# AHupuJR/REFID

Hardware: AMD Instinct MI355X
Metric: interpolated frames/sec (train step) GoPro 256x256 11+1 (higher is better)
Workload: dtype f32

## Files before the change

### refid_amd/csrc/conv_wino6.hip

```cpp
#include "common.h"
#include "conv_args.h"
#include <algorithm>
#include <cstdlib>

#ifndef REFID_WINO6_ABLATE
#define REFID_WINO6_ABLATE 0
#endif

namespace {

constexpr int TW = 32;
constexpr int KC = 16;
constexpr int HWD = TW + 2;
constexpr int TH = 4;
constexpr int ROWP = 40;
constexpr int PLANE = 6 * ROWP + 5;
constexpr int R_F4 = 4 * PLANE;
constexpr int HP = (TH + 2) * HWD;
constexpr int R_ITEMS = (4 * HP + 255) / 256;
constexpr int lds_bytes(int nt) { return nt == 2 ? 64 * 66 * 16 : (32 * 66 * 16 > 2 * R_F4 * 16 ? 32 * 66 * 16 : 2 * R_F4 * 16); }
constexpr int OOB = -1;
typedef __bf16 bf16x8 __attribute__((ext_vector_type(8)));
typedef _Float16 f16x8 __attribute__((ext_vector_type(8)));
typedef _Float16 f16x2 __attribute__((ext_vector_type(2)));
typedef float f32x2 __attribute__((ext_vector_type(2)));
constexpr int W3H_HEADER = 64;
constexpr int F16_TGT = 7;
constexpr int F16_SLACK = 6;
constexpr int F16_E0 = F16_TGT + 1;

__device__ __forceinline__ void split8(const f32x4& v0, const f32x4& v1, f32x4 (&pl)[3]) {
    bf16x8 p0, p1, p2;
#pragma unroll
    for (int k = 0; k < 8; ++k) {
        const float v = k < 4 ? v0[k] : v1[k - 4];
        const __bf16 h = (__bf16)v;
        p0[k] = h;
        const float r = v - (float)h;
        const __bf16 m = (__bf16)r;
        p1[k] = m;
        p2[k] = (__bf16)(r - (float)m);
    }
    pl[0] = __builtin_bit_cast(f32x4, p0);
    pl[1] = __builtin_bit_cast(f32x4, p1);
    pl[2] = __builtin_bit_cast(f32x4, p2);
}

__device__ __forceinline__ void split8h(const f32x4& v0, const f32x4& v1, f32x4 (&pl)[3]) {
    f16x8 h, l;
#pragma unroll
    for (int k = 0; k < 8; k += 2) {
        const f32x2 ab = {k < 4 ? v0[k] : v1[k - 4], k < 4 ? v0[k + 1] : v1[k - 3]};
        const f16x2 hh = __builtin_convertvector(ab, f16x2);
        const f32x2 r = ab - __builtin_convertvector(hh, f32x2);
        const f16x2 ll = __builtin_convertvector(r, f16x2);
        h[k] = hh[0]; h[k + 1] = hh[1];
        l[k] = ll[0]; l[k + 1] = ll[1];
    }
    pl[0] = __builtin_bit_cast(f32x4, h);
    pl[1] = __builtin_bit_cast(f32x4, l);
}

template <int NT, bool F16>
__global__ __launch_bounds__(256, NT == 2 ? 2 : 3) void conv_wino6_kernel(const ConvKArgs a) {
    constexpr int BN = 32 * NT;
    constexpr int NPL = F16 ? 2 : 3;
    constexpr int NPR = (REFID_WINO6_ABLATE == 14 || REFID_WINO6_ABLATE == 15) ? 3 : (F16 ? 3 : 6);
    extern __shared__ __attribute__((aligned(16))) char smem[];
    f32x4* sR = reinterpret_cast<f32x4*>(smem);

    const int tid = threadIdx.x;
    const int lane = tid & 63, wave = tid >> 6;
    const int li = lane & 31, kh = lane >> 5;
    const int ti = wave;
    if (REFID_WINO6_ABLATE == 20 && a.N > 0) return;
    if (REFID_WINO6_ABLATE == 21 && a.N > 0) { __syncthreads(); if (tid == 12345) a.out[0] = 1.f; return; }

#if defined(REFID_WINO6_ABLATE) && (REFID_WINO6_ABLATE == 9 || REFID_WINO6_ABLATE == 11)
    {
        unsigned hw;
        asm volatile("s_getreg_b32 %0, hwreg(HW_REG_HW_ID)" : "=s"(hw));
        if ((hw & 1) && blockIdx.x < 512 * 2) {
            const unsigned long long t0 = wall_clock64();
            while (wall_clock64() - t0 < (REFID_WINO6_ABLATE == 9 ? 400 : 800)) __builtin_amdgcn_s_sleep(8);
        }
    }
#endif
    const int xcd = blockIdx.x & 7, slot = blockIdx.x >> 3;
    int bt = (slot / a.ncot) * 8 + xcd;
    if (bt >= a.tilesX * a.tilesY * a.N) return;
    const int n0 = (slot % a.ncot) * BN;
    const int tx = bt % a.tilesX; bt /= a.tilesX;
    const int ty = bt % a.tilesY;
    const int n = bt / a.tilesY;
    const int oy0 = ty * TH, ox0 = tx * TW;

    const int limA = (int)min((long long)a.N * a.H * a.W * a.ldA * 4, 0x7fffffffLL);
    const int limB = a.inB ? (int)min((long long)a.N * a.H * a.W * a.ldB * 4, 0x7fffffffLL) : 0;
    const int uPlane = a.CoutPad * KC * 2;
    const int uXi = NPL * uPlane;
    const int uChunk = 16 * uXi;
    const __amdgpu_buffer_rsrc_t rsW = __builtin_amdgcn_make_buffer_rsrc(
        const_cast<float*>(a.w) + (F16 ? W3H_HEADER / 4 : 0), 0, (int)min((long long)a.nchunks * uChunk, 0x7fffffffLL), 0x00020000);
    const int eU = F16 ? *reinterpret_cast<const int*>(a.w) : 0;
    int eRef = F16_E0;
    const int q = tid & 3;
    int pixo[R_ITEMS], sdst[R_ITEMS];
#pragma unroll
    for (int it = 0; it < R_ITEMS; ++it) {
        const int hp = (tid >> 2) + it * 64;
        const int row = hp / HWD, col = hp % HWD;
        const int iy = oy0 - a.pad + row, ix = ox0 - a.pad + col;
        const bool ok = hp < HP && iy >= 0 && iy < a.H && ix >= 0 && ix < a.W;
        pixo[it] = ok ? (n * a.H + iy) * a.W + ix : OOB;
        sdst[it] = hp < HP ? q * PLANE + row * ROWP + (col >> 1) + (col & 1) * 20 : q * PLANE + 6 * ROWP + (tid & 3);
    }
    int voU[NT];
#pragma unroll
    for (int nt = 0; nt < NT; ++nt) {
        const int urow = a.coBase + n0 + nt * 32 + li;
        voU[nt] = (urow < a.CoutPad) ? (urow * KC + kh * 8) * 2 + ti * 4 * uXi : OOB;
        if (REFID_WINO6_ABLATE == 12) voU[nt] = ti * 4 * uXi;
    }
    const int kper = (a.nchunks + a.ksplit - 1) / a.ksplit;
    const int kc0 = blockIdx.y * kper, kc1 = min(a.nchunks, kc0 + kper);

    f32x4 rr[R_ITEMS];
    auto load_raw = [&](int ch, f32x4 (&dst)[R_ITEMS]) {
        const int c0 = (REFID_WINO6_ABLATE == 5 ? 0 : ch) * KC;
        const bool fromA = c0 < a.Ca;
        const int soff = (fromA ? c0 : c0 - a.Ca) * 4;
        const int qmask = (ch < kc1 && c0 + q * 4 < a.Ctot) ? 0 : OOB;
        const int ld4 = (fromA ? a.ldA : a.ldB) * 4;
        const __amdgpu_buffer_rsrc_t rs = __builtin_amdgcn_make_buffer_rsrc(
            const_cast<float*>(fromA ? a.inA : a.inB), 0, fromA ? limA : limB, 0x00020000);
#pragma unroll
        for (int it = 0; it < R_ITEMS; ++it) {
            const int vo = (pixo[it] * ld4 + q * 16) | qmask;
            dst[it] = __builtin_bit_cast(f32x4, __builtin_amdgcn_raw_buffer_load_b128(rs, vo, soff, 0));
        }
    };
    auto store_raw = [&](int buf, const f32x4 (&src)[R_ITEMS]) {
#pragma unroll
        for (int it = 0; it < R_ITEMS; ++it) sR[buf * R_F4 + sdst[it]] = src[it];
    };
    auto load_u = [&](int ch, int j, f32x4 (&dst)[NPL][NT]) {
        const bool in = ch < kc1;
        const int so = (REFID_WINO6_ABLATE == 1 ? 0 : ch) * uChunk + j * uXi;
#pragma unroll
        for (int p = 0; p < ((REFID_WINO6_ABLATE == 14 || REFID_WINO6_ABLATE == 15) ? 2 : NPL); ++p)
#pragma unroll
            for (int nt = 0; nt < NT; ++nt) {
                if (REFID_WINO6_ABLATE == 13 && nt == 1) { dst[p][nt] = dst[p][0]; continue; }
                dst[p][nt] = __builtin_bit_cast(
                    f32x4, __builtin_amdgcn_raw_buffer_load_b128(rsW, in ? voU[nt] : OOB, in ? so + p * uPlane : 0, 0));
            }
    };

    f32x16 acc[4][NT];
#pragma unroll
    for (int j = 0; j < 4; ++j)
#pragma unroll
        for (int t = 0; t < NT; ++t)
#pragma unroll
            for (int r = 0; r < 16; ++r) acc[j][t][r] = 0.f;

    const int rowP = (ti == 0) ? 0 : ((ti == 2) ? 2 : 1);
    const int rowM = (ti == 0) ? 2 : ((ti == 1) ? 2 : ((ti == 2) ? 1 : 3));
    const float sgn = (ti == 1) ? 1.f : -1.f;
    const int tbase = 2 * kh * PLANE + (2 * (li >> 4)) * ROWP + (li & 15);
    const int offP = tbase + rowP * ROWP, offM = tbase + rowM * ROWP;
    constexpr int BOFF[4] = {0, 20, 1, 21};

    constexpr int TA[6] = {0, 0, 1, 0, 2, 1};
    constexpr int TB[6] = {0, 1, 0, 2, 0, 1};

    f32x4 uA[NPL][NT], uB[NPL][NT];
    auto phase = [&](int ch) {
        const int lc = ch - kc0;
        if (REFID_WINO6_ABLATE != 7 && REFID_WINO6_ABLATE != 8) {
            store_raw((lc + 1) & 1, rr);
            load_raw(ch + 2, rr);
#ifdef REFID_WINO6_PIN
            __builtin_amdgcn_sched_barrier(0x38F);
#endif
        }
        const f32x4* r = sR + (lc & 1) * R_F4;
        f32x4 t[2][4];
#pragma unroll
        for (int qq = 0; qq < 2; ++qq)
#pragma unroll
            for (int b = 0; b < 4; ++b) t[qq][b] = r[qq * PLANE + offP + BOFF[b]] + r[qq * PLANE + offM + BOFF[b]] * sgn;
        if constexpr (F16 && REFID_WINO6_ABLATE != 16) {
            float m = 0.f;
#pragma unroll
            for (int qq = 0; qq < 2; ++qq)
#pragma unroll
                for (int b = 0; b < 4; ++b)
                    m = fmaxf(fmaxf(m, fmaxf(fabsf(t[qq][b][0]), fabsf(t[qq][b][1]))), fmaxf(fabsf(t[qq][b][2]), fabsf(t[qq][b][3])));
            if (REFID_WINO6_ABLATE == 17) m = fabsf(t[0][0][0]);
            const unsigned mb = __float_as_uint(m);
            const auto sw = __builtin_amdgcn_permlane32_swap(mb, mb, false, false);
            const int eb = (int)(max(sw[0], sw[1]) >> 23);
            const bool grow = eb > eRef + F16_SLACK;
            if (__builtin_amdgcn_ballot_w64(grow) != 0) {
                const int en = grow ? eb : eRef;
                const int fe = 127 + eRef - en;
                const float f = fe >= 1 ? __uint_as_float((unsigned)fe << 23) : 0.f;
#pragma unroll
                for (int j = 0; j < 4; ++j)
#pragma unroll
                    for (int nt = 0; nt < NT; ++nt)
#pragma unroll
                        for (int rr2 = 0; rr2 < 16; ++rr2) acc[j][nt][rr2] *= f;
                eRef = en;
            }
            const float sc = __uint_as_float((unsigned)(F16_TGT + 254 - eRef) << 23);
#pragma unroll
            for (int qq = 0; qq < 2; ++qq)
#pragma unroll
                for (int b = 0; b < 4; ++b) t[qq][b] *= sc;
        }
#pragma unroll
        for (int j = 0; j < 4; ++j) {
            f32x4 (&cur)[NPL][NT] = (j & 1) ? uB : uA;
            f32x4 (&nxt)[NPL][NT] = (j & 1) ? uA : uB;
            if (REFID_WINO6_ABLATE != 6 && REFID_WINO6_ABLATE != 8) load_u(j == 3 ? ch + 1 : ch, (j + 1) & 3, nxt);
#ifdef REFID_WINO6_PIN
            __builtin_amdgcn_sched_barrier(0x38F);
#endif
            f32x4 v[2], pl[3];
#pragma unroll
            for (int qq = 0; qq < 2; ++qq)
                v[qq] = (j == 0) ? t[qq][0] - t[qq][2] : (j == 1) ? t[qq][1] + t[qq][2]
                      : (j == 2) ? t[qq][2] - t[qq][1] : t[qq][1] - t[qq][3];
            if (REFID_WINO6_ABLATE == 2 || REFID_WINO6_ABLATE == 15) { pl[0] = v[0]; pl[1] = v[1]; pl[2] = t[0][j]; }
            else if (F16 && REFID_WINO6_ABLATE == 18) { pl[0] = v[0]; pl[1] = v[1]; }
            else if constexpr (F16) split8h(v[0], v[1], pl);
            else split8(v[0], v[1], pl);
#pragma unroll
            for (int e = 0; e < NPR; ++e)
#pragma unroll
                for (int nt = 0; nt < NT; ++nt) {
                    if constexpr (F16)
                        acc[j][nt] = __builtin_amdgcn_mfma_f32_32x32x16_f16(
                            __builtin_bit_cast(f16x8, cur[TB[e]][nt]), __builtin_bit_cast(f16x8, pl[TA[e]]), acc[j][nt], 0, 0, 0);
                    else
                        acc[j][nt] = __builtin_amdgcn_mfma_f32_32x32x16_bf16(
                            __builtin_bit_cast(bf16x8, cur[TB[e]][nt]), __builtin_bit_cast(bf16x8, pl[TA[e]]), acc[j][nt], 0, 0, 0);
                }
        }
        __syncthreads();
    };

    {
        f32x4 rr0[R_ITEMS];
#if REFID_WINO6_ABLATE == 19
        int keep[R_ITEMS];
#pragma unroll
        for (int it = 0; it < R_ITEMS; ++it) {
            keep[it] = pixo[it];
            const int hp = (tid >> 2) + it * 64;
            const int row = hp / HWD, col = hp % HWD;
            pixo[it] = (hp < HP && row >= a.pad && col >= a.pad) ? (row - a.pad) * a.W + (col - a.pad) : OOB;
        }
#endif
        load_raw(kc0, rr0);
        load_raw(kc0 + 1, rr);
#if REFID_WINO6_ABLATE == 19
#pragma unroll
        for (int it = 0; it < R_ITEMS; ++it) pixo[it] = keep[it];
#endif
        load_u(kc0, 0, uA);
        if (REFID_WINO6_ABLATE == 6 || REFID_WINO6_ABLATE == 8) load_u(kc0, 1, uB);
        store_raw(0, rr0);
    }
    __syncthreads();

    if (REFID_WINO6_ABLATE != 3 && REFID_WINO6_ABLATE != 10)
        for (int ch = kc0; ch < kc1; ++ch) phase(ch);

    constexpr int XL = 66;
    f32x4* xch = reinterpret_cast<f32x4*>(smem);
#pragma unroll
    for (int t = 0; t < NT; ++t)
#pragma unroll
        for (int rq = 0; rq < 4; ++rq) {
            f32x4 r0, r1;
#pragma unroll
            for (int k = 0; k < 4; ++k) {
                const int r = 4 * rq + k;
                r0[k] = acc[0][t][r] + acc[1][t][r] + acc[2][t][r];
                r1[k] = acc[1][t][r] - acc[2][t][r] - acc[3][t][r];
                if constexpr (F16) {
                    r0[k] = ldexpf(r0[k], eRef - 127 - F16_TGT - eU);
                    r1[k] = ldexpf(r1[k], eRef - 127 - F16_TGT - eU);
                }
            }
            xch[(((ti * 2 + 0) * NT + t) * 4 + rq) * XL + kh * 33 + li] = r0;
            xch[(((ti * 2 + 1) * NT + t) * 4 + rq) * XL + kh * 33 + li] = r1;
        }
    constexpr int QUADS = BN / 4, PPT = 256 / QUADS, CPR = TW / PPT;
    constexpr int NIT = TH * CPR;
    static_assert(TW == 32 && (NT == 1 || NT == 2) && PPT * CPR == TW, "epilogue item mapping");
    constexpr int TI_STRIDE = 2 * NT * 4 * XL;
    const int p0 = tid / QUADS, c = (tid % QUADS) * 4;
    const int j0 = n0 + c;
    const int nt = c >> 5, rq = (c & 31) >> 3, ckh = (c & 7) >> 2;
    const long long opb = (long long)(n * a.Ho + oy0) * a.Wo + ox0 + p0;
    const bool jok = j0 < a.Cout;
    const bool vec = a.vecOK && (j0 + 3 < a.Cout);
    bool cok[CPR];
#pragma unroll
    for (int q2 = 0; q2 < CPR; ++q2) cok[q2] = ox0 + q2 * PPT + p0 < a.Wo;
    float* const outB = a.out + (a.ksplit > 1 ? blockIdx.y * a.wsStride : 0) + opb * a.ldO + j0;
    const float* const resB = a.res ? a.res + opb * a.ldR + j0 : nullptr;
    const float* const mskB = a.mask ? a.mask + opb * a.ldM + j0 : nullptr;
    const int stepO[2] = {a.Wo * a.ldO, PPT * a.ldO}, stepR[2] = {a.Wo * a.ldR, PPT * a.ldR}, stepM[2] = {a.Wo * a.ldM, PPT * a.ldM};
    const bool two = a.out2 != nullptr && a.ksplit == 1;
    float* const out2B = two ? a.out2 + opb * a.ldO2 + j0 : nullptr;
    const float* const add2B = two ? a.add2 + opb * a.ldA2 + j0 : nullptr;
    const int stepO2[2] = {a.Wo * a.ldO2, PPT * a.ldO2}, stepA2[2] = {a.Wo * a.ldA2, PPT * a.ldA2};
    const bool pre = REFID_WINO6_ABLATE != 4 && REFID_WINO6_ABLATE != 10 && vec && a.ksplit == 1 && (a.res != nullptr || a.mask != nullptr);
    f32x4 pres[NIT], pmask[NIT];
    if (pre) {
#pragma unroll
        for (int it = 0; it < NIT; ++it) {
            const bool ok = (oy0 + it / CPR < a.Ho) && cok[it % CPR];
            pres[it] = f32x4{0.f, 0.f, 0.f, 0.f};
            pmask[it] = f32x4{1.f, 1.f, 1.f, 1.f};
            if (ok && a.res) pres[it] = *reinterpret_cast<const f32x4*>(resB + (it / CPR) * stepR[0] + (it % CPR) * stepR[1]);
            if (ok && a.mask) pmask[it] = *reinterpret_cast<const f32x4*>(mskB + (it / CPR) * stepM[0] + (it % CPR) * stepM[1]);
        }
    }
    f32x4 bv = {0.f, 0.f, 0.f, 0.f};
    if (a.bias && a.ksplit == 1 && jok) {
        const float* bp = a.bias + a.coBase + j0;
        if (vec) bv = *reinterpret_cast<const f32x4*>(bp);
        else
#pragma unroll
            for (int k = 0; k < 4; ++k) if (j0 + k < a.Cout) bv[k] = bp[k];
    }
    __syncthreads();

#pragma unroll
    for (int it = 0; it < NIT; ++it) {
        const int row = it / CPR, colb = it % CPR;
        const int col = colb * PPT + p0;
        const int oa = row & 1, tile = ((row & 3) >> 1) * 16 + (col >> 1), ob = col & 1;
        if (oy0 + row >= a.Ho || !cok[colb] || !jok) continue;
        const f32x4* xp = xch + (((oa * 2 + ob) * NT + nt) * 4 + rq) * XL + ckh * 33 + tile;
        const float sg = oa ? -1.f : 1.f;
        f32x4 v = xp[0] + (xp[TI_STRIDE] + xp[2 * TI_STRIDE]) * sg;
        float* const outp = outB + row * stepO[0] + colb * stepO[1];
        if (a.ksplit > 1) {
            *reinterpret_cast<f32x4*>(outp) = v;
            continue;
        }
        v += bv;
        lrelu4(v, a.slopePre, a.slopePre != 1.f);
        if (REFID_WINO6_ABLATE == 4 || REFID_WINO6_ABLATE == 10) {
            if (v[0] == 12345.678f) outp[0] = v[1];
            continue;
        }
        if (vec) {
            if (a.res) v += pre ? pres[it] : *reinterpret_cast<const f32x4*>(resB + row * stepR[0] + colb * stepR[1]);
            lrelu4(v, a.slopePost, a.slopePost != 1.f);
            if (a.mask) {
                const f32x4 mv = pre ? pmask[it] : *reinterpret_cast<const f32x4*>(mskB + row * stepM[0] + colb * stepM[1]);
#pragma unroll
                for (int k = 0; k < 4; ++k) v[k] *= (mv[k] > 0.f) ? 1.f : a.slopeMask;
            }
            *reinterpret_cast<f32x4*>(outp) = v;
            if (two)
                *reinterpret_cast<f32x4*>(out2B + row * stepO2[0] + colb * stepO2[1]) =
                    v + *reinterpret_cast<const f32x4*>(add2B + row * stepA2[0] + colb * stepA2[1]);
        } else {
#pragma unroll
            for (int k = 0; k < 4; ++k) {
                if (j0 + k >= a.Cout) break;
                float tv = v[k];
                if (a.res) tv += resB[row * stepR[0] + colb * stepR[1] + k];
                tv = lrelu(tv, a.slopePost);
                if (a.mask) tv *= (mskB[row * stepM[0] + colb * stepM[1] + k] > 0.f) ? 1.f : a.slopeMask;
                outp[k] = tv;
                if (two) out2B[row * stepO2[0] + colb * stepO2[1] + k] = tv + add2B[row * stepA2[0] + colb * stepA2[1] + k];
            }
        }
    }
}

struct Wino6Plan { int ks; int nt; dim3 grid; };

Wino6Plan wino6_plan(ConvKArgs& a, int split_mode, int tile_hint = 0) {
    Wino6Plan p;
    p.nt = (a.Cout > 32 && tile_hint != 4) ? 2 : 1;
    a.tilesX = cdiv(a.Wo, TW);
    a.tilesY = cdiv(a.Ho, TH);
    if (p.nt == 2 && tile_hint == 0 && split_mode) {
        const int ncot2 = cdiv(a.Cout, 64);
        const int nwg2 = (split_mode == 2) ? round_up(a.tilesX * a.tilesY * a.N, 8) * ncot2 : a.tilesX * a.tilesY * ncot2 * 8;
        static const int small_wg = []() { const char* e = getenv("REFID_WINO6_SMALL"); return e ? atoi(e) : 512; }();
        static const int small_k = []() { const char* e = getenv("REFID_WINO6_SMALL_K"); return e ? atoi(e) : 9; }();
        if (nwg2 <= small_wg && cdiv(a.Ctot, KC) < small_k) p.nt = 1;
    }
    const int bn = 32 * p.nt;
    a.nchunks = cdiv(a.Ctot, KC);
    a.ncot = cdiv(a.Cout, bn);
    p.grid = dim3(round_up(a.tilesX * a.tilesY * a.N, 8) * a.ncot);
    const int nwg = (split_mode == 2) ? (int)p.grid.x : a.tilesX * a.tilesY * a.ncot * 8;
    int ks = 1;
    if (split_mode && nwg <= 256 && a.nchunks >= 8) {
        ks = 512 / nwg;
        if (ks > a.nchunks / 4) ks = a.nchunks / 4;
        if (ks > 8) ks = 8;
        if (ks < 1) ks = 1;
    }
    p.ks = ks;
    return p;
}

template <int NT, bool F16>
int launch_wino6_t(const ConvKArgs& a, dim3 grid, hipStream_t st, const char* what) {
    static std::atomic<unsigned long long> done{0};
    if (int rc = refid_lds_attr_once(done, &conv_wino6_kernel<NT, F16>, lds_bytes(NT), "conv_wino6")) return rc;
    hipLaunchKernelGGL((conv_wino6_kernel<NT, F16>), grid, dim3(256), lds_bytes(NT), st, a);
    REFID_LAUNCH_CHECK(what);
    return 0;
}

template <int NT>
int launch_wino6(const ConvKArgs& a, bool f16, dim3 grid, hipStream_t st, const char* what) {
    return f16 ? launch_wino6_t<NT, true>(a, grid, st, what) : launch_wino6_t<NT, false>(a, grid, st, what);
}

}

bool refid_wino6_eligible(const ConvKArgs& a) {
    const long long lim = 0x7fffffffLL;
    return a.Cout >= 1 && a.Ctot % 4 == 0 && (a.inB == nullptr || a.Ca % KC == 0) &&
           (long long)a.N * a.H * a.W * a.ldA * 4 < lim && (!a.inB || (long long)a.N * a.H * a.W * a.ldB * 4 < lim) &&
           (long long)cdiv(a.Ctot, KC) * 16 * 3 * a.CoutPad * KC * 2 < lim;
}

size_t refid_wino6_workspace_bytes(const ConvKArgs& ka, int split_mode) {
    size_t need = 0;
    for (int hint : {0, 1, 4}) {
        ConvKArgs a = ka;
        const Wino6Plan p = wino6_plan(a, split_mode, hint);
        if (p.ks > 1) need = std::max(need, (size_t)p.ks * a.N * a.Ho * a.Wo * round_up(a.Cout, 4) * sizeof(float));
    }
    return need;
}

int refid_launch_wino6(const ConvKArgs& ka, float* ws, size_t ws_bytes, int split_mode, int tile_hint, int terms, hipStream_t st) {
    ConvKArgs a = ka;
    REFID_CHECK(terms == 0 || terms == 6 || terms == 3, "conv2d: algo 5 takes mfma_terms 0 / 6 (six bf16 products) or 3 (three fp16 "
                "products, w_packed from refid_pack_conv_weights_wino3h), got %d", terms);
    const bool f16 = terms == 3;
    REFID_CHECK(!f16 || (reinterpret_cast<uintptr_t>(a.w) & 15) == 0, "conv2d: the fp16 Winograd packing must be 16-byte aligned");
    REFID_CHECK(refid_wino6_eligible(a),
                "conv2d: the Winograd six-product tile needs input-channel counts that are multiples "
                "of 4 (two sources: c_a a multiple of 16) and tensors below 2 GiB");
    const Wino6Plan pl = wino6_plan(a, ws ? split_mode : 0, tile_hint);
    dim3 grid = pl.grid;
    const int ks = pl.ks;
    if (ks == 1) return pl.nt == 2 ? launch_wino6<2>(a, f16, grid, st, "conv_wino6") : launch_wino6<1>(a, f16, grid, st, "conv_wino6/32");
    const long long npix = (long long)a.N * a.Ho * a.Wo;
    const int ldW = round_up(a.Cout, 4);
    const size_t need = (size_t)ks * npix * ldW * sizeof(float);
    if (need > ws_bytes || (reinterpret_cast<uintptr_t>(ws) & 15)) {
        refid_set_error("conv_wino6: split-K workspace too small or misaligned (%zu bytes given, %zu needed: "
                        "refid_conv_workspace_bytes)", ws_bytes, need);
        return 1;
    }
    ConvKArgs p = a;
    p.ksplit = ks; p.wsStride = npix * ldW; p.out = ws; p.ldO = ldW; p.out2 = nullptr;
    grid.y = ks;
    if (int rc = pl.nt == 2 ? launch_wino6<2>(p, f16, grid, st, "conv_wino6/splitk") : launch_wino6<1>(p, f16, grid, st, "conv_wino6/32/splitk"))
        return rc;
    ConvKArgs f = a;
    f.ksplit = ks; f.wsStride = npix * ldW;
    return refid_launch_splitk_finish(f, ws, ldW, npix, st);
}
```

Baseline: 518.5.

## Stream Winograd input halos straight into LDS via buffer-load-to-LDS ring

For the 64-wide output tile, the input halo is now loaded with buffer_load ... lds (direct global-to-LDS DMA) into a four-deep ring, with a swizzled slot layout, instead of passing through registers and being stored to LDS by hand. The halo loads are issued mid-loop, and chunk boundaries wait on vmcnt with a per-wave barrier rather than a full __syncthreads. This is meant to cut VGPR pressure and the LDS store instructions and to deepen the prefetch. It adds a new LDS layout with XOR swizzling and hand-tuned waitcnt counts, which are a correctness risk. An optional three-set weight-register rotation is also added.

```diff
diff --git a/refid_amd/csrc/conv_wino6.hip b/refid_amd/csrc/conv_wino6.hip
--- a/refid_amd/csrc/conv_wino6.hip
+++ b/refid_amd/csrc/conv_wino6.hip
@@ -2,6 +2,7 @@
 #include "conv_args.h"
 #include <algorithm>
 #include <cstdlib>
+#include <type_traits>
 
 #ifndef REFID_WINO6_ABLATE
 #define REFID_WINO6_ABLATE 0
@@ -20,6 +21,20 @@
 constexpr int R_ITEMS = (4 * HP + 255) / 256;
 constexpr int lds_bytes(int nt) { return nt == 2 ? 64 * 66 * 16 : (32 * 66 * 16 > 2 * R_F4 * 16 ? 32 * 66 * 16 : 2 * R_F4 * 16); }
 constexpr int OOB = -1;
+constexpr int DROWP = 36;
+constexpr int DSLOTS = 6 * DROWP;
+constexpr int DRING = 4;
+constexpr int DBUF_F4 = 1024;
+constexpr int DPIECES = 4;
+static_assert(4 * DSLOTS <= DPIECES * 256 && DPIECES * 256 == DBUF_F4 && DRING * DBUF_F4 * 16 <= lds_bytes(2), "halo ring");
+typedef __attribute__((address_space(3))) void* lds_ptr24;
+constexpr int vmcnt_lgkm0(int nn) { return (nn & 15) | ((nn >> 4) << 14) | 0x0070; }
+#ifndef REFID_WINO6_USETS
+#define REFID_WINO6_USETS 2
+#endif
+#ifndef REFID_WINO6_HALO_AT
+#define REFID_WINO6_HALO_AT 3
+#endif
 typedef __bf16 bf16x8 __attribute__((ext_vector_type(8)));
 typedef _Float16 f16x8 __attribute__((ext_vector_type(8)));
 typedef _Float16 f16x2 __attribute__((ext_vector_type(2)));
@@ -61,7 +76,7 @@
     pl[1] = __builtin_bit_cast(f32x4, l);
 }
 
-template <int NT, bool F16>
+template <int NT, bool F16, bool DMA>
 __global__ __launch_bounds__(256, NT == 2 ? 2 : 3) void conv_wino6_kernel(const ConvKArgs a) {
     constexpr int BN = 32 * NT;
     constexpr int NPL = F16 ? 2 : 3;
@@ -104,16 +119,25 @@
         const_cast<float*>(a.w) + (F16 ? W3H_HEADER / 4 : 0), 0, (int)min((long long)a.nchunks * uChunk, 0x7fffffffLL), 0x00020000);
     const int eU = F16 ? *reinterpret_cast<const int*>(a.w) : 0;
     int eRef = F16_E0;
-    const int q = tid & 3;
-    int pixo[R_ITEMS], sdst[R_ITEMS];
-#pragma unroll
-    for (int it = 0; it < R_ITEMS; ++it) {
+    const int q = DMA ? (tid & 3) ^ ((tid >> 4) & 3) : tid & 3;
+    constexpr int NREQ = DMA ? DPIECES : R_ITEMS;
+    int pixo[NREQ], sdst[DMA ? 1 : R_ITEMS];
+    auto halo_pixel = [&](int it, int nn, int y0, int x0) {
         const int hp = (tid >> 2) + it * 64;
-        const int row = hp / HWD, col = hp % HWD;
-        const int iy = oy0 - a.pad + row, ix = ox0 - a.pad + col;
-        const bool ok = hp < HP && iy >= 0 && iy < a.H && ix >= 0 && ix < a.W;
-        pixo[it] = ok ? (n * a.H + iy) * a.W + ix : OOB;
-        sdst[it] = hp < HP ? q * PLANE + row * ROWP + (col >> 1) + (col & 1) * 20 : q * PLANE + 6 * ROWP + (tid & 3);
+        const int row = DMA ? hp / DROWP : hp / HWD;
+        const int col = DMA ? hp - row * DROWP - ((row >> 1) & 1) : hp % HWD;
+        const int iy = y0 + row, ix = x0 + col;
+        const bool ok = (DMA ? row < 6 && col >= 0 && col < HWD : hp < HP) && iy >= 0 && iy < a.H && ix >= 0 && ix < a.W;
+        return ok ? (nn * a.H + iy) * a.W + ix : OOB;
+    };
+#pragma unroll
+    for (int it = 0; it < NREQ; ++it) {
+        pixo[it] = halo_pixel(it, n, oy0 - a.pad, ox0 - a.pad);
+        if constexpr (!DMA) {
+            const int hp = (tid >> 2) + it * 64;
+            const int row = hp / HWD, col = hp % HWD;
+            sdst[it] = hp < HP ? q * PLANE + row * ROWP + (col >> 1) + (col & 1) * 20 : q * PLANE + 6 * ROWP + (tid & 3);
+        }
     }
     int voU[NT];
 #pragma unroll
@@ -125,8 +149,8 @@
     const int kper = (a.nchunks + a.ksplit - 1) / a.ksplit;
     const int kc0 = blockIdx.y * kper, kc1 = min(a.nchunks, kc0 + kper);
 
-    f32x4 rr[R_ITEMS];
-    auto load_raw = [&](int ch, f32x4 (&dst)[R_ITEMS]) {
+    f32x4 rr[DMA ? 1 : R_ITEMS];
+    auto load_raw = [&](int ch, f32x4 (&dst)[DMA ? 1 : R_ITEMS]) {
         const int c0 = (REFID_WINO6_ABLATE == 5 ? 0 : ch) * KC;
         const bool fromA = c0 < a.Ca;
         const int soff = (fromA ? c0 : c0 - a.Ca) * 4;
@@ -134,15 +158,17 @@
         const int ld4 = (fromA ? a.ldA : a.ldB) * 4;
         const __amdgpu_buffer_rsrc_t rs = __builtin_amdgcn_make_buffer_rsrc(
             const_cast<float*>(fromA ? a.inA : a.inB), 0, fromA ? limA : limB, 0x00020000);
-#pragma unroll
-        for (int it = 0; it < R_ITEMS; ++it) {
+        char* const ring = smem + ((ch - kc0) & (DRING - 1)) * (DBUF_F4 * 16) + __builtin_amdgcn_readfirstlane(wave) * 1024;
+#pragma unroll
+        for (int it = 0; it < NREQ; ++it) {
             const int vo = (pixo[it] * ld4 + q * 16) | qmask;
-            dst[it] = __builtin_bit_cast(f32x4, __builtin_amdgcn_raw_buffer_load_b128(rs, vo, soff, 0));
+            if constexpr (DMA) __builtin_amdgcn_raw_ptr_buffer_load_lds(rs, (lds_ptr24)(ring + it * 4096), 16, vo, soff, 0, 0);
+            else dst[it] = __builtin_bit_cast(f32x4, __builtin_amdgcn_raw_buffer_load_b128(rs, vo, soff, 0));
         }
     };
-    auto store_raw = [&](int buf, const f32x4 (&src)[R_ITEMS]) {
-#pragma unroll
-        for (int it = 0; it < R_ITEMS; ++it) sR[buf * R_F4 + sdst[it]] = src[it];
+    auto store_raw = [&](int buf, const f32x4 (&src)[DMA ? 1 : R_ITEMS]) {
+#pragma unroll
+        for (int it = 0; it < (DMA ? 0 : R_ITEMS); ++it) sR[buf * R_F4 + sdst[it]] = src[it];
     };
     auto load_u = [&](int ch, int j, f32x4 (&dst)[NPL][NT]) {
         const bool in = ch < kc1;
@@ -171,26 +197,47 @@
     const int tbase = 2 * kh * PLANE + (2 * (li >> 4)) * ROWP + (li & 15);
     const int offP = tbase + rowP * ROWP, offM = tbase + rowM * ROWP;
     constexpr int BOFF[4] = {0, 20, 1, 21};
+    int rdo[2][4];
+    if constexpr (DMA) {
+#pragma unroll
+        for (int x = 0; x < 2; ++x)
+#pragma unroll
+            for (int b = 0; b < 4; ++b) {
+                const int row = (x ? rowM : rowP) + 2 * (li >> 4);
+                const int sl = row * DROWP + ((row >> 1) & 1) + 2 * (li & 15) + b;
+                rdo[x][b] = sl * 4 + ((2 * kh) ^ ((sl >> 2) & 3));
+            }
+    }
+    constexpr int ULD = (REFID_WINO6_ABLATE == 6 || REFID_WINO6_ABLATE == 8) ? 0
+                      : ((REFID_WINO6_ABLATE == 14 || REFID_WINO6_ABLATE == 15) ? 2 : NPL) * (REFID_WINO6_ABLATE == 13 ? 1 : NT);
+    constexpr int HLD = (REFID_WINO6_ABLATE == 7 || REFID_WINO6_ABLATE == 8) ? 0 : DPIECES;
+    constexpr int VM_KEEP = 4 * ULD + 2 * HLD;
 
     constexpr int TA[6] = {0, 0, 1, 0, 2, 1};
     constexpr int TB[6] = {0, 1, 0, 2, 0, 1};
 
-    f32x4 uA[NPL][NT], uB[NPL][NT];
-    auto phase = [&](int ch) {
+    constexpr int NSETS = (DMA && REFID_WINO6_USETS == 3) ? 3 : 2;
+    f32x4 us[NSETS][NPL][NT];
+    auto phase = [&](int ch, auto pc) {
+        constexpr int P = decltype(pc)::value;
         const int lc = ch - kc0;
-        if (REFID_WINO6_ABLATE != 7 && REFID_WINO6_ABLATE != 8) {
+        if (!DMA && REFID_WINO6_ABLATE != 7 && REFID_WINO6_ABLATE != 8) {
             store_raw((lc + 1) & 1, rr);
             load_raw(ch + 2, rr);
 #ifdef REFID_WINO6_PIN
             __builtin_amdgcn_sched_barrier(0x38F);
 #endif
         }
-        const f32x4* r = sR + (lc & 1) * R_F4;
+        if (DMA && HLD && REFID_WINO6_HALO_AT < 0) load_raw(ch + DRING - 1, rr);
+        const f32x4* r = sR + (DMA ? (lc & (DRING - 1)) * DBUF_F4 : (lc & 1) * R_F4);
         f32x4 t[2][4];
 #pragma unroll
         for (int qq = 0; qq < 2; ++qq)
 #pragma unroll
-            for (int b = 0; b < 4; ++b) t[qq][b] = r[qq * PLANE + offP + BOFF[b]] + r[qq * PLANE + offM + BOFF[b]] * sgn;
+            for (int b = 0; b < 4; ++b) {
+                if constexpr (DMA) t[qq][b] = r[rdo[0][b] ^ qq] + r[rdo[1][b] ^ qq] * sgn;
+                else t[qq][b] = r[qq * PLANE + offP + BOFF[b]] + r[qq * PLANE + offM + BOFF[b]] * sgn;
+            }
         if constexpr (F16 && REFID_WINO6_ABLATE != 16) {
             float m = 0.f;
 #pragma unroll
@@ -223,9 +270,15 @@
         }
 #pragma unroll
         for (int j = 0; j < 4; ++j) {
-            f32x4 (&cur)[NPL][NT] = (j & 1) ? uB : uA;
-            f32x4 (&nxt)[NPL][NT] = (j & 1) ? uA : uB;
-            if (REFID_WINO6_ABLATE != 6 && REFID_WINO6_ABLATE != 8) load_u(j == 3 ? ch + 1 : ch, (j + 1) & 3, nxt);
+            f32x4 (&cur)[NPL][NT] = us[(P + j) % NSETS];
+            f32x4 (&nxt)[NPL][NT] = us[(P + j + NSETS - 1) % NSETS];
+            if (REFID_WINO6_ABLATE != 6 && REFID_WINO6_ABLATE != 8)
+                load_u(j + NSETS - 1 > 3 ? ch + 1 : ch, (j + NSETS - 1) & 3, nxt);
+            if (DMA && HLD && j == REFID_WINO6_HALO_AT) {
+                __builtin_amdgcn_sched_barrier(0x38F);
+                load_raw(ch + DRING - 1, rr);
+                __builtin_amdgcn_sched_barrier(0x38F);
+            }
 #ifdef REFID_WINO6_PIN
             __builtin_amdgcn_sched_barrier(0x38F);
 #endif
@@ -250,35 +303,69 @@
                             __builtin_bit_cast(bf16x8, cur[TB[e]][nt]), __builtin_bit_cast(bf16x8, pl[TA[e]]), acc[j][nt], 0, 0, 0);
                 }
         }
+        if constexpr (DMA) {
+            constexpr int keep = vmcnt_lgkm0(VM_KEEP);
+            __builtin_amdgcn_s_waitcnt(keep);
+            __builtin_amdgcn_s_barrier();
+        } else
+            __syncthreads();
+    };
+
+    {
+        f32x4 rr0[DMA ? 1 : R_ITEMS];
+#if REFID_WINO6_ABLATE == 19
+        int keep[NREQ];
+#pragma unroll
+        for (int it = 0; it < NREQ; ++it) {
+            keep[it] = pixo[it];
+            pixo[it] = halo_pixel(it, 0, -a.pad, -a.pad);
+        }
+#endif
+        load_raw(kc0, rr0);
+        if constexpr (DMA) {
+            load_u(kc0, 0, us[0]);
+            if (NSETS == 3 || REFID_WINO6_ABLATE == 6 || REFID_WINO6_ABLATE == 8) load_u(kc0, 1, us[1]);
+            load_raw(kc0 + 1, rr);
+            load_raw(kc0 + 2, rr);
+        } else
+            load_raw(kc0 + 1, rr);
+#if REFID_WINO6_ABLATE == 19
+#pragma unroll
+        for (int it = 0; it < NREQ; ++it) pixo[it] = keep[it];
+#endif
+        if constexpr (!DMA) {
+            load_u(kc0, 0, us[0]);
+            if (REFID_WINO6_ABLATE == 6 || REFID_WINO6_ABLATE == 8) load_u(kc0, 1, us[1]);
+            store_raw(0, rr0);
+        }
+    }
+    if constexpr (DMA) {
+        constexpr int keep = vmcnt_lgkm0(2 * DPIECES);
+        __builtin_amdgcn_s_waitcnt(keep);
+        __builtin_amdgcn_s_barrier();
+    } else
         __syncthreads();
-    };
-
+
+    if (REFID_WINO6_ABLATE != 3 && REFID_WINO6_ABLATE != 10)
     {
-        f32x4 rr0[R_ITEMS];
-#if REFID_WINO6_ABLATE == 19
-        int keep[R_ITEMS];
-#pragma unroll
-        for (int it = 0; it < R_ITEMS; ++it) {
-            keep[it] = pixo[it];
-            const int hp = (tid >> 2) + it * 64;
-            const int row = hp / HWD, col = hp % HWD;
-            pixo[it] = (hp < HP && row >= a.pad && col >= a.pad) ? (row - a.pad) * a.W + (col - a.pad) : OOB;
-        }
-#endif
-        load_raw(kc0, rr0);
-        load_raw(kc0 + 1, rr);
-#if REFID_WINO6_ABLATE == 19
-#pragma unroll
-        for (int it = 0; it < R_ITEMS; ++it) pixo[it] = keep[it];
-#endif
-        load_u(kc0, 0, uA);
-        if (REFID_WINO6_ABLATE == 6 || REFID_WINO6_ABLATE == 8) load_u(kc0, 1, uB);
-        store_raw(0, rr0);
-    }
-    __syncthreads();
-
-    if (REFID_WINO6_ABLATE != 3 && REFID_WINO6_ABLATE != 10)
-        for (int ch = kc0; ch < kc1; ++ch) phase(ch);
+        using P0 = std::integral_constant<int, 0>;
+        if constexpr (NSETS == 3) {
+            int ch = kc0;
+            for (; ch + 2 < kc1; ch += 3) {
+                phase(ch, P0{});
+                phase(ch + 1, std::integral_constant<int, 1>{});
+                phase(ch + 2, std::integral_constant<int, 2>{});
+            }
+            if (ch < kc1) phase(ch, P0{});
+            if (ch + 1 < kc1) phase(ch + 1, std::integral_constant<int, 1>{});
+        } else
+            for (int ch = kc0; ch < kc1; ++ch) phase(ch, P0{});
+    }
+    if constexpr (DMA) {
+        constexpr int none = vmcnt_lgkm0(0);
+        __builtin_amdgcn_s_waitcnt(none);
+        __builtin_amdgcn_s_barrier();
+    }
 
     constexpr int XL = 66;
     f32x4* xch = reinterpret_cast<f32x4*>(smem);
@@ -390,11 +477,12 @@
     }
 }
 
-struct Wino6Plan { int ks; int nt; dim3 grid; };
+struct Wino6Plan { int ks; int nt; bool dma; dim3 grid; };
 
 Wino6Plan wino6_plan(ConvKArgs& a, int split_mode, int tile_hint = 0) {
     Wino6Plan p;
     p.nt = (a.Cout > 32 && tile_hint != 4) ? 2 : 1;
+    if (tile_hint == 5) tile_hint = 0;
     a.tilesX = cdiv(a.Wo, TW);
     a.tilesY = cdiv(a.Ho, TH);
     if (p.nt == 2 && tile_hint == 0 && split_mode) {
@@ -404,6 +492,7 @@
         static const int small_k = []() { const char* e = getenv("REFID_WINO6_SMALL_K"); return e ? atoi(e) : 9; }();
         if (nwg2 <= small_wg && cdiv(a.Ctot, KC) < small_k) p.nt = 1;
     }
+    p.dma = p.nt == 2;
     const int bn = 32 * p.nt;
     a.nchunks = cdiv(a.Ctot, KC);
     a.ncot = cdiv(a.Cout, bn);
@@ -420,18 +509,19 @@
     return p;
 }
 
-template <int NT, bool F16>
+template <int NT, bool F16, bool DMA>
 int launch_wino6_t(const ConvKArgs& a, dim3 grid, hipStream_t st, const char* what) {
     static std::atomic<unsigned long long> done{0};
-    if (int rc = refid_lds_attr_once(done, &conv_wino6_kernel<NT, F16>, lds_bytes(NT), "conv_wino6")) return rc;
-    hipLaunchKernelGGL((conv_wino6_kernel<NT, F16>), grid, dim3(256), lds_bytes(NT), st, a);
+    if (int rc = refid_lds_attr_once(done, &conv_wino6_kernel<NT, F16, DMA>, lds_bytes(NT), "conv_wino6")) return rc;
+    hipLaunchKernelGGL((conv_wino6_kernel<NT, F16, DMA>), grid, dim3(256), lds_bytes(NT), st, a);
     REFID_LAUNCH_CHECK(what);
     return 0;
 }
 
-template <int NT>
-int launch_wino6(const ConvKArgs& a, bool f16, dim3 grid, hipStream_t st, const char* what) {
-    return f16 ? launch_wino6_t<NT, true>(a, grid, st, what) : launch_wino6_t<NT, false>(a, grid, st, what);
+int launch_wino6(const ConvKArgs& a, int nt, bool dma, bool f16, dim3 grid, hipStream_t st, const char* what) {
+    if (nt == 1) return f16 ? launch_wino6_t<1, true, false>(a, grid, st, what) : launch_wino6_t<1, false, false>(a, grid, st, what);
+    if (dma) return f16 ? launch_wino6_t<2, true, true>(a, grid, st, what) : launch_wino6_t<2, false, true>(a, grid, st, what);
+    return f16 ? launch_wino6_t<2, true, false>(a, grid, st, what) : launch_wino6_t<2, false, false>(a, grid, st, what);
 }
 
 }
@@ -445,7 +535,7 @@
 
 size_t refid_wino6_workspace_bytes(const ConvKArgs& ka, int split_mode) {
     size_t need = 0;
-    for (int hint : {0, 1, 4}) {
+    for (int hint : {0, 1, 4, 5}) {
         ConvKArgs a = ka;
         const Wino6Plan p = wino6_plan(a, split_mode, hint);
         if (p.ks > 1) need = std::max(need, (size_t)p.ks * a.N * a.Ho * a.Wo * round_up(a.Cout, 4) * sizeof(float));
@@ -465,7 +555,8 @@
     const Wino6Plan pl = wino6_plan(a, ws ? split_mode : 0, tile_hint);
     dim3 grid = pl.grid;
     const int ks = pl.ks;
-    if (ks == 1) return pl.nt == 2 ? launch_wino6<2>(a, f16, grid, st, "conv_wino6") : launch_wino6<1>(a, f16, grid, st, "conv_wino6/32");
+    const bool dma = pl.dma && tile_hint != 5;
+    if (ks == 1) return launch_wino6(a, pl.nt, dma, f16, grid, st, pl.nt == 2 ? "conv_wino6" : "conv_wino6/32");
     const long long npix = (long long)a.N * a.Ho * a.Wo;
     const int ldW = round_up(a.Cout, 4);
     const size_t need = (size_t)ks * npix * ldW * sizeof(float);
@@ -477,8 +568,7 @@
     ConvKArgs p = a;
     p.ksplit = ks; p.wsStride = npix * ldW; p.out = ws; p.ldO = ldW; p.out2 = nullptr;
     grid.y = ks;
-    if (int rc = pl.nt == 2 ? launch_wino6<2>(p, f16, grid, st, "conv_wino6/splitk") : launch_wino6<1>(p, f16, grid, st, "conv_wino6/32/splitk"))
-        return rc;
+    if (int rc = launch_wino6(p, pl.nt, dma, f16, grid, st, pl.nt == 2 ? "conv_wino6/splitk" : "conv_wino6/32/splitk")) return rc;
     ConvKArgs f = a;
     f.ksplit = ks; f.wsStride = npix * ldW;
     return refid_launch_splitk_finish(f, ws, ldW, npix, st);
```

New measurement: 520.7 (median of 6 runs). Within noise of the previous version (+0.4%).
